# bdagnillo/altair-raytracing

Hardware: AMD Instinct MI355X
Metric: Mrays/sec whole-node, 180x90 fluxmap src(-60,0,-75); achieved HBM GB/s vs peak (higher is better)
Workload: dtype f64

## Files before the change

### altair-raytracing_amd/csrc/isx_api.hip

```cpp
#include "../../include/isx.h"
#include "isx_kernels.hpp"

#include <cmath>
#include <cstdio>
#include <cstdlib>
#include <cstring>
#include <algorithm>
#include <limits>
#include <map>
#include <new>
#include <tuple>
#include <variant>
#include <vector>

using namespace isx;

namespace {

struct State {
  bool init = false;
  int device = -1;
  int cu_count = 0;
  size_t lds_limit = 64 * 1024;
  hipStream_t stream = nullptr;
// ... 3178 lines not shown

int isx_scene_path_moments(const isx_scene_path_spec* pspec, const uint64_t* hist, const isx_scene_path_counts* counts,
                           double* mean_cm, double* sd_cm) {
  if (!pspec || !hist || !counts) return ISX_ERR_BAD_ARG;
  const int rc = check_scene_path_spec(pspec);
  if (rc) return rc;
  const size_t K = (size_t)pspec->n_bins;
  for (int f = 0; f < ISX_RESPONSE_FATES; ++f) {
    const uint64_t* row = hist + (size_t)f * K;
    double N = 0, A = 0, B = 0;
    for (size_t k = 0; k < K; ++k) {
      const double h = (double)row[k], x = ((double)k + 0.5) * pspec->bin_cm;
      N += h;
      A += x * h;
      B += x * x * h;
    }
    double m = std::numeric_limits<double>::quiet_NaN(), d = m;
    if (N > 0 && counts->overflow[f] == 0) {
      m = A / N;
      const double var = B / N - m * m;
      d = std::sqrt(var > 0 ? var : 0.0);
    }
    if (mean_cm) mean_cm[f] = m;
    if (sd_cm) sd_cm[f] = d;
  }
  return ISX_OK;
}

int isx_scene_path_decay(const isx_scene_path_spec* pspec, const uint64_t* hist, const isx_scene_path_counts* counts, int32_t f,
                         int32_t lo_bin, double* tau_cm, double* sigma_cm) {
  if (!pspec || !hist || !counts || !tau_cm || !sigma_cm) return ISX_ERR_BAD_ARG;
  const int rc = check_scene_path_spec(pspec);
  if (rc) return rc;
  if (f < 0 || f >= ISX_RESPONSE_FATES || lo_bin < 0 || lo_bin >= pspec->n_bins) return ISX_ERR_BAD_ARG;
  if (counts->overflow[f] != 0) return ISX_ERR_BAD_CONFIG;
  const uint64_t* row = hist + (size_t)f * (size_t)pspec->n_bins;
  double N = 0, Sm = 0;
  for (int32_t ib = lo_bin; ib < pspec->n_bins; ++ib) {
    const double h = (double)row[ib];
    Sm += (double)(ib - lo_bin) * h;
    N += h;
  }
  if (!(N > 0)) return ISX_ERR_BAD_CONFIG;
  const double m = Sm / N;
  if (!(m > 0)) return ISX_ERR_BAD_CONFIG;
  const double r = m / (1.0 + m);
  const double lr = std::log(r);
  *tau_cm = -pspec->bin_cm / lr;
  *sigma_cm = pspec->bin_cm / (lr * lr) / std::sqrt(N * m * (1.0 + m));
  return ISX_OK;
}

#ifdef ISX_DIAG
int isx_diag_read(uint64_t* out48) {
  if (!S.init || !out48) return ISX_ERR_BAD_ARG;
  if (trace_join()) return ISX_ERR_HIP;
  HIPCHK(hipStreamSynchronize(S.stream));
  HIPCHK(hipMemcpyFromSymbol(out48, HIP_SYMBOL(isx::g_diag), 48 * sizeof(unsigned long long)));
  unsigned long long z[48] = {0};
  HIPCHK(hipMemcpyToSymbol(HIP_SYMBOL(isx::g_diag), z, sizeof(z)));
  return ISX_OK;
}
#endif

}
```

### altair-raytracing_amd/csrc/isx_kernels.hpp

```cpp
#pragma once
#include <type_traits>
#include "isx_device.hpp"

namespace isx {

struct DetGrid {
  int n_theta, n_phi, nbins, bin_mode;
  int hit_line_mode, pad0;
  double half_w2;
  double rho_d;
  double R;
  double portz;
  const double* table;
  const double* rowtab;
  const double* coltab;
  const double* discs;
  double disc_r, disc_h;
  const float* clusters;
  const int* disc_perm;
  int n_clusters, pad1;
  uint64_t map_first, rays_per_group;
  int fold;
  int rec_stage;
  double* rec_lines;
  uint32_t* rec_counts;
  double* log_rec;
  unsigned long long* log_count;
  uint64_t log_cap;
  int xm_nu, xm_nv, xm_nx, xm_ny;
  double xm_plane_z, xm_half;
  unsigned long long* xm_dir;
  unsigned long long* xm_pos;
  unsigned long long* xm_counts;
};

#ifdef ISX_DIAG
__device__ unsigned long long g_diag[48];
#define ISX_DIAG_ADD(k, v) do { if (lane == 0) atomicAdd(&g_diag[k], (unsigned long long)(v)); } while (0)
#define ISX_DIAG_ADD_LANES(k, v) atomicAdd(&g_diag[k], (unsigned long long)(v))
#define ISX_TD_DECL unsigned long long td_[16] = {0}; unsigned long long tdc_ = clock64()
#define ISX_TD_MARK(k) do { const unsigned long long c_ = clock64(); td_[k] += c_ - tdc_; tdc_ = c_; } while (0)
#define ISX_TD_ADD(k, v) do { td_[k] += (unsigned long long)(v); } while (0)
#define ISX_TD_FLUSH() do { if (lane == 0) for (int k_ = 0; k_ < 16; ++k_) atomicAdd(&g_diag[16 + k_], td_[k_]); } while (0)
#define ISX_TD_FLUSH_AT(b_) do { if (lane == 0) for (int k_ = 0; k_ < 16; ++k_) atomicAdd(&g_diag[(b_) + k_], td_[k_]); } while (0)
#define ISX_BD_MARK(sq, k) do { if (lane == 0) { const unsigned long long c_ = clock64(); \
    const unsigned long long p_ = ((unsigned long long)(unsigned)(sq).head[7] << 32) | (unsigned)(sq).tail[7]; \
    atomicAdd(&g_diag[16 + (k)], c_ - p_); (sq).tail[7] = (int)(unsigned)c_; (sq).head[7] = (int)(unsigned)(c_ >> 32); } } while (0)
#define ISX_BD_INIT(sq) do { if (lane == 0) { const unsigned long long c_ = clock64(); (sq).tail[7] = (int)(unsigned)c_; (sq).head[7] = (int)(unsigned)(c_ >> 32); } } while (0)
#else
#define ISX_BD_INIT(sq) do { } while (0)
#define ISX_BD_MARK(sq, k) do { } while (0)
#define ISX_DIAG_ADD(k, v) do { } while (0)
#define ISX_DIAG_ADD_LANES(k, v) do { } while (0)
#define ISX_TD_DECL do { } while (0)
#define ISX_TD_MARK(k) do { } while (0)
#define ISX_TD_ADD(k, v) do { } while (0)
#define ISX_TD_FLUSH() do { } while (0)
#define ISX_TD_FLUSH_AT(b_) do { } while (0)
#endif

enum : int { SINK_FLUX = 0, SINK_DZ = 1, SINK_DISC = 2, SINK_PERPOS = 3, SINK_LOG = 4, SINK_DISCPOS = 5, SINK_REC = 6, SINK_EXITMAP = 7, SINK_WALL = 8,
              SINK_LIGHTFIELD = 9, SINK_ORDER = 10, SINK_PATCH = 11,
              SINK_RESPONSE = 12,
              SINK_VIEW = 13,
              SINK_FIELD = 14,
              SINK_SORDER = 15,
              SINK_SPATH = 16 };

struct Work {
  uint64_t seed, first, n;
  unsigned long long* hist;
  unsigned long long* stats;
  uint32_t* ctr;
  uint32_t sub, pad;
};
enum : int { Q_RAYS = 0 , Q_REGIONS = 2, Q_BIN = 3,
             Q_SCAN = 4 , Q_LIST = 6, Q_LISTB = 7, Q_WORDS = 8 };
constexpr uint32_t kRegion = 1024;

#ifndef ISX_BLOCK
#define ISX_BLOCK 1024
#endif
#ifndef ISX_WAVES_PER_EU
#define ISX_WAVES_PER_EU 0
#endif
constexpr int kBlock = ISX_BLOCK;
#ifndef ISX_ABL
#define ISX_ABL 0
#endif
#ifndef ISX_WALK4
#define ISX_WALK4 1
#endif
#ifndef ISX_ATOM_BRANCH
#define ISX_ATOM_BRANCH 0
#endif
#ifndef ISX_ASSIST_MIN
#define ISX_ASSIST_MIN 64
#endif
#ifndef ISX_ASSIST_LAZY
#define ISX_ASSIST_LAZY 128
#endif
// ... 651 lines not shown
        const int slot = lane >> logq;
        part = lane & ((1 << logq) - 1);
        have = slot < nlong;
        const int e = have ? ((volatile LdsInt*)split)[slot] : 0;
        owner = e & 63;
        i = e >> 8;
      }
      if (!have) i = 0;
      CapWin w;
      w.inv_dphi = inv_dphi;
      w.Fz = __shfl(pre.Fz, owner, 64); w.AF = __shfl(pre.AF, owner, 64); w.AF2 = w.AF * w.AF;
      w.jf = __shfl(pre.jf, owner, 64); w.ch2 = __shfl(pre.ch2, owner, 64);
      V3 P, V;
      {
        load_line(lines + 6 * owner, P, V);
      }
      int jlo = 0, cnt = 0;
      if (have) cap_window(w, (float)rowt[4 * i + 2], (float)rowt[4 * i + 3], d.n_phi, jlo, cnt);
      int start = 0, len = cnt;
      if (pass == 0) {
        const unsigned long long lm = __ballot(cnt > kSplitAt);
        if (lm != 0ull && __ballot(cnt >= kSplitAt + 16) != 0ull) {
          nlong = (int)__popcll(lm);
          logq = nlong <= 8 ? 3 : (nlong <= 16 ? 2 : (nlong <= 32 ? 1 : 0));
          if (logq > 0) {
            npass = 2;
            if (cnt > kSplitAt) {
              const uint32_t rank = __builtin_amdgcn_mbcnt_hi((uint32_t)(lm >> 32), __builtin_amdgcn_mbcnt_lo((uint32_t)lm, 0u));
              ((volatile LdsInt*)split)[rank] = owner | (i << 8);
              len = kSplitAt;
            }
            __builtin_amdgcn_wave_barrier();
          }
        }
      } else {
        const int rem = cnt - kSplitAt;
        const int chunk = (rem + (1 << logq) - 1) >> logq;
        start = kSplitAt + part * chunk;
        len = rem - part * chunk;
        len = len < 0 ? 0 : (len > chunk ? chunk : len);
        if (!have) len = 0;
      }
      ISX_DIAG_ADD(11, 1); if (pass == 1) ISX_DIAG_ADD(10, 1);
      const double t0 = -fma(P.x, V.x, fma(P.y, V.y, (P.z - d.portz) * V.z));
      walk_columns(d, hist, colx, P, V, t0, lane, i, rowt, jlo, start, len, 0, lines + 6 * owner);
    }
  }
}

constexpr int kClasses = 7, kQueueCap = 128;
constexpr int kSlotWaveWords = kClasses * kQueueCap + 16 + 64;
constexpr int kDeferCap = kDeferCapW;
constexpr int kDeferHead = 8;
constexpr int kColWaveWords = kClasses * kQueueCap + 16 + 64 + kDeferHead + kDeferCap;
constexpr int kPiece = 16, kLongest = 24;
struct SlotQueues {
  LdsWord* q;
  LdsInt* tail;
  LdsInt* head;
  const ColP* colp;
  LdsWord* defer;
};
__device__ __forceinline__ const uint2* defer_side(const SlotQueues& sq) {
  volatile LdsWord* df = sq.defer;
  return reinterpret_cast<const uint2*>((uintptr_t)((unsigned long long)df[1] | ((unsigned long long)df[2] << 32)));
}
__device__ __forceinline__ uint2 side_load(const uint2* side, int i) {
  const unsigned long long w = ((__attribute__((address_space(1))) const unsigned long long*)side)[i];
  return make_uint2((uint32_t)w, (uint32_t)(w >> 32));
}
__device__ __forceinline__ void redo_push(const SlotQueues& sq, uint32_t id, uint32_t bin) {
  volatile LdsWord* df = sq.defer;
  GlbU64* redo = (GlbU64*)(uintptr_t)((unsigned long long)df[4] | ((unsigned long long)df[5] << 32));
  const unsigned long long cap = (unsigned long long)df[6] | ((unsigned long long)df[7] << 32);
  const unsigned long long pos = __hip_atomic_fetch_add(redo, 1ull, __ATOMIC_RELAXED, __HIP_MEMORY_SCOPE_AGENT);
  if (pos < cap) redo[2ull + pos] = (unsigned long long)id | ((unsigned long long)bin << 32);
  else redo[1] = 1ull;
}
__device__ __forceinline__ int slot_class(int cnt) {
  return cnt <= 4 ? 0 : (cnt <= 12 ? (cnt - 3) >> 1 : (cnt <= 16 ? 5 : 6));
}

constexpr uint32_t kDeferFlushAt = 64;
template <class D>
__device__ __forceinline__ void flush_deferred(const D& d, uint32_t* __restrict__ hist, const double* __restrict__ rowt,
                                               const ColX* __restrict__ colx, const double* __restrict__ lines, const SlotQueues& sq,
                                               int lane) {
  volatile LdsWord* df = sq.defer;
  typedef __attribute__((address_space(3))) uint32_t LdsU32;
  const uint32_t held = df[0];
  const uint32_t n = held < (uint32_t)kDeferCap ? held : (uint32_t)kDeferCap;
#pragma unroll 1
  for (uint32_t base = 0; base < n; base += 64u) {
    const bool have = base + (uint32_t)lane < n;
    const uint32_t e = have ? df[(uint32_t)kDeferHead + base + (uint32_t)lane] : 0u;
    const int line = (int)(e & 255u), jr = (int)((e >> 8) & 255u), ir = (int)((e >> 16) & 255u);
    bool hit = false;
    const uint2* side = defer_side(sq);
    if (side) {
      uint2 se = make_uint2(0u, 0u);
      if (have) se = side_load(side, line);
      const float e = __uint_as_float(se.x);
      int res = 0;
      if (have) res = e > 0.f ? decide_approx(d, rowt, colx, lines + 6 * line, ir, jr, e) : (int)decide_exact(d, rowt, colx, lines + 6 * line, ir, jr);
      hit = res == 1;
      const unsigned long long rm = __ballot(res == 2);
      if (rm) {
// ... 147 lines not shown
  ilo = max((int)floorf((thF - omega) * k.inv_dth - 0.5f - 1e-3f), 0);
  ihi = min((int)ceilf((thF + omega) * k.inv_dth - 0.5f + 1e-3f), k.n_theta - 1);
  own.smax = Gz; own.smin = AF; own.vxy = phiF * k.inv_dphi - 0.5f; own.avz = ch2;
}

template <class D>
__device__ __forceinline__ void produce_rows_packed(const D& d, uint32_t* __restrict__ hist, const double* __restrict__ rowt,
                                                    const ColX* __restrict__ colx, const double* __restrict__ lines, const SlotQueues& sq,
                                                    const BoxLine& own, int own_ilo, int nrow, int excl, int incl, int total, bool boxes,
                                                    float inv_dphi, float portz, int first_line, int lane, LdsInt* mark) {
#pragma unroll 1
  for (int base = 0; base < total; base += 64) {
    const int g = base + lane;
    bool have = g < total;
    volatile LdsInt* mk = mark;
    mk[lane] = 0;
    __builtin_amdgcn_wave_barrier();
    if (nrow > 0 && excl < base + 64 && incl > base) mk[(excl > base ? excl : base) - base] = lane + 1;
    __builtin_amdgcn_wave_barrier();
    const int m = mk[lane];
    const unsigned long long low = __ballot(m != 0) & (~0ull >> (63 - lane));
    const int pos = 63 - __builtin_clzll(low | 1ull);
    int owner = mk[pos] - 1;
    if (!have || owner < 0) { owner = 0; have = false; }
    const int o_excl = __shfl(excl, owner, 64), o_ilo = __shfl(own_ilo, owner, 64);
    BoxLine b;
    b.smax = __shfl(own.smax, owner, 64); b.smin = __shfl(own.smin, owner, 64); b.vxy = __shfl(own.vxy, owner, 64);
    b.avz = __shfl(own.avz, owner, 64);
    b.ivz = b.dn = b.Hm = b.Hz = b.phin = b.rs = b.sig = 0.f;
    if (boxes) {
      b.ivz = __shfl(own.ivz, owner, 64); b.dn = __shfl(own.dn, owner, 64); b.Hm = __shfl(own.Hm, owner, 64);
      b.Hz = __shfl(own.Hz, owner, 64); b.phin = __shfl(own.phin, owner, 64); b.rs = __shfl(own.rs, owner, 64);
      b.sig = __shfl(own.sig, owner, 64);
    }
    const int i = have ? o_ilo + (g - o_excl) : 0;
    int j0 = 0, c0 = 0, j1 = 0, c1 = 0;
    if (have) {
      const float zi = (float)rowt[4 * i + 2], Ai = (float)rowt[4 * i + 3];
      if (boxes) box_window(b, zi - portz, Ai, d.n_phi, inv_dphi, j0, c0, j1, c1);
      else {
        CapWin w;
        w.inv_dphi = inv_dphi; w.Fz = b.smax; w.AF = b.smin; w.AF2 = b.smin * b.smin; w.jf = b.vxy; w.ch2 = b.avz;
        cap_window(w, zi, Ai, d.n_phi, j0, c0);
      }
    }
    const int nwin = (boxes && __ballot(c1 > 0) != 0ull) ? 2 : 1;
#pragma unroll 1
    for (int w = 0; w < nwin; ++w) push_slots(d, hist, rowt, colx, lines, sq, first_line + owner, i, w == 0 ? j0 : j1, w == 0 ? c0 : c1, lane);
  }
}

struct __align__(16) RowX { float S0, S1, C0, C1, T0, T1; uint32_t pad0, pad1; };
constexpr int kColPiece = 48, kColLongest = 64;
__device__ __forceinline__ int col_class(int cnt) { return cnt <= 48 ? (cnt - 1) >> 3 : 6; }

struct ColPre {
  float fx, fy, a, cosw;
  int jlo, ncol;
  int kind;
};
__device__ __forceinline__ ColPre prep_cols(const GridConst& k, int n_phi, const V3& P, const V3& V, const CapShared& sh, int side) {
  ColPre o;
  o.fx = o.fy = o.a = o.cosw = 0.f; o.jlo = 0; o.ncol = 0; o.kind = sh.kind;
  if (sh.kind != 0) return o;
  float Fx, Fy, mz;
  cap_centre(k, sh, P, V, side, Fx, Fy, mz);
  if (mz * sh.iL * k.Rf - sqrt_cull(cap_chord2(k, sh)) > 0.f) { o.kind = -3; return o; }
  o.fx = Fx * sh.iL; o.fy = Fy * sh.iL; o.a = -(mz * sh.iL);
  o.cosw = sh.cosw;
  o.kind = 0;
  const float sinF = sqrt_cull(fmaf(o.fx, o.fx, o.fy * o.fy));
  const float sinw = sqrt_cull(fmaxf(0.f, fmaf(-o.cosw, o.cosw, 1.0f)));
  if (!(sinF > sinw * 1.01f + 1e-4f)) { o.jlo = 0; o.ncol = n_phi; return o; }
  const float r = fminf(1.0f, sinw * rcp_cull(sinF) * 1.001f);
  const float dphi = (1.57079637f - acos_cull(r)) + 3e-3f;
  float phiF = atan2_cull(Fy, Fx);
  if (phiF < 0.f) phiF += 6.28318530718f;
  const float jc = phiF * k.inv_dphi - 0.5f, hw = dphi * k.inv_dphi + 0.02f;
  const int lo = (int)ceilf(jc - hw), hi = (int)floorf(jc + hw);
  int n = hi - lo + 1;
  if (n >= n_phi) { o.jlo = 0; o.ncol = n_phi; return o; }
  if (n < 0) n = 0;
  int j0 = lo;
  if (j0 < 0) j0 += n_phi;
  if (j0 >= n_phi) j0 -= n_phi;
  o.jlo = j0; o.ncol = n;
  return o;
}

__device__ __forceinline__ void cap_rows(float fx, float fy, float a, float cosw, float c32, float s32, float inv_dth, int n_theta,
                                         int& ilo, int& cnt) {
#if ISX_ABL == 3
  ilo = 20; cnt = 30; return;
#endif
  ilo = 0; cnt = 0;
  const float b = fmaf(c32, fx, s32 * fy);
  const float rho2 = fmaf(a, a, b * b);
  if (!(rho2 > 1e-12f)) { if (cosw < 1e-5f) cnt = n_theta; return; }
  const float x = cosw * __builtin_amdgcn_rsqf(rho2);
  if (x > 1.0f) return;
  if (x < 0.0f) { ilo = 0; cnt = n_theta; return; }
  const float dl = acos_cull(fmaxf(x, -1.0f)) + 2.5e-3f;
  const float tc = atan2_cull(b, a);
  const float tlo = tc - dl, thi = tc + dl;
  if (thi < 0.f || tlo > 1.57079637f) return;
  const int lo = max((int)ceilf(tlo * inv_dth - 0.5f - 1e-3f), 0);
  const int hi = min((int)floorf(thi * inv_dth - 0.5f + 1e-3f), n_theta - 1);
// ... 27 lines not shown
    ex = fmaf(-tv, Vx, tx); ey = fmaf(-tv, Vy, ty); ez = fmaf(-tv, Vz, tz);
    const float ie = __builtin_amdgcn_rsqf(fmaf(ex, ex, fmaf(ey, ey, ez * ez)));
    ex *= ie; ey *= ie; ez *= ie;
    cosw = -1.0f;
  }
  o.fx = ex; o.fy = ey; o.a = -ez; o.cosw = cosw; o.kind = 0;
  bp.ux = fmaf(Vy, ez, -(Vz * ey)); bp.uy = fmaf(Vz, ex, -(Vx * ez)); bp.uz = fmaf(Vx, ey, -(Vy * ex));
  bp.kap = fmaf(rs * iR, 1.0001f, 4e-6f) + kap_extra;
  const float sinF = sqrt_cull(fmaf(o.fx, o.fx, o.fy * o.fy));
  const float sinw = sqrt_cull(fmaxf(0.f, fmaf(-cosw, cosw, 1.0f)));
  if (!(cosw > 0.05f) || !(sinF > sinw * 1.01f + 1e-4f)) { o.jlo = 0; o.ncol = n_phi; return o; }
  const float r = fminf(1.0f, sinw * rcp_cull(sinF) * 1.001f);
  const float dphi = (1.57079637f - acos_cull(r)) + 3e-3f;
  float phiF = atan2_cull(o.fy, o.fx);
  if (phiF < 0.f) phiF += 6.28318530718f;
  const float jc = phiF * k.inv_dphi - 0.5f, hw = dphi * k.inv_dphi + 0.02f;
  const int lo = (int)ceilf(jc - hw), hi = (int)floorf(jc + hw);
  int n = hi - lo + 1;
  if (n >= n_phi) { o.jlo = 0; o.ncol = n_phi; return o; }
  if (n < 0) n = 0;
  int j0 = lo;
  if (j0 < 0) j0 += n_phi;
  if (j0 >= n_phi) j0 -= n_phi;
  o.jlo = j0; o.ncol = n;
  return o;
}
__device__ __forceinline__ void band_rows(const BandPre& bp, float c32, float s32, float inv_dth, int row_lo, int row_hi, int& ilo, int& cnt,
                                          int& ilo_b, int& cnt_b) {
  ilo = cnt = ilo_b = cnt_b = 0;
  if (row_hi < row_lo) return;
  const float ga = fmaf(c32, bp.ux, s32 * bp.uy);
  const float N2 = fmaf(ga, ga, bp.uz * bp.uz);
  if (!(N2 > bp.kap * bp.kap * 1.03f + 1e-12f)) { ilo = row_lo; cnt = row_hi - row_lo + 1; return; }
  const float x = bp.kap * __builtin_amdgcn_rsqf(N2);
  const float al = (1.57079637f - acos_cull(x)) + 2.6e-3f;
  const float de = atan2_cull(bp.uz, ga);
#pragma unroll
  for (int m = -1; m <= 1; ++m) {
    const float ce = fmaf((float)m, 3.14159274f, de);
    const float tlo = ce - al, thi = ce + al;
    if (thi < 0.f || tlo > 1.57079637f) continue;
    const int lo = max((int)ceilf(tlo * inv_dth - 0.5f - 1e-3f), row_lo);
    const int hi = min((int)floorf(thi * inv_dth - 0.5f + 1e-3f), row_hi);
    if (hi < lo) continue;
    if (cnt == 0) { ilo = lo; cnt = hi - lo + 1; }
    else { ilo_b = lo; cnt_b = hi - lo + 1; }
  }
}

template <class D>
__device__ __forceinline__ void consume_cols(const D& d, uint32_t* __restrict__ hist, const double* __restrict__ rowt,
                                             const ColX* __restrict__ colx, const RowX* __restrict__ rowx,
                                             const double* __restrict__ lines, uint32_t rec, bool active, int lane,
                                             const SlotQueues& sq) {
  ISX_BD_MARK(sq, 3);
#if ISX_ABL == 2
  return;
#endif
  const int line = (int)(rec & 255u), j = (int)((rec >> 8) & 255u), ilo = (int)((rec >> 16) & 255u);
  const int len = active ? (int)(rec >> 24) : 0;
  const double* src6 = lines + 6 * line;
  float cAl = 0.f, cBe = 0.f, cVz = 0.f, cQz = 0.f, cE0 = 0.f, cE1 = 0.f, cE2 = 0.f, cF0 = 0.f, cF1 = 0.f, cF2 = 0.f;
  float band32 = 0.f;
  if (len > 0) {
    V3 P, V;
    {
      load_line(src6, P, V);
    }
    const double wz = P.z - d.portz;
    const double t0 = -fma(P.x, V.x, fma(P.y, V.y, wz * V.z));
    const double qx = fma(t0, V.x, P.x), qy = fma(t0, V.y, P.y), qz = fma(t0, V.z, wz);
    const double cph = colx[j].c, sph = colx[j].s;
    const double al = fma(V.y, cph, -(V.x * sph)), be = fma(qy, cph, -(qx * sph));
    const double ga = fma(V.x, cph, V.y * sph), de = fma(qx, cph, qy * sph);
    const double R = d.R, R2x = 2.0 * R;
    const double e0 = -2.0 * fma(qx, V.x, fma(qy, V.y, qz * V.z));
    const double f0 = fma(qx, qx, fma(qy, qy, fma(qz, qz, R * R))) - d.half_w2;
    const double e1 = R2x * ga, e2 = -(R2x * V.z), f1 = -(R2x * de), f2 = R2x * qz;
    cAl = (float)al; cBe = (float)be; cVz = (float)(-V.z); cQz = (float)(-qz);
    cE0 = (float)e0; cF0 = (float)f0; cE1 = (float)e1; cF1 = (float)f1; cE2 = (float)e2; cF2 = (float)f2;
    const double Md = fabs(al) + fabs(V.z), Mn = fabs(be) + (fabs(qz) + R);
    const double Mv = fabs(e0) + (fabs(e1) + fabs(e2)), Mf = fabs(f0) + (fabs(f1) + fabs(f2));
    const double Sg = fma(Md, fma(Md, Mf, Mn * Mv), Mn * Mn);
    band32 = Sg >= 1e-6 ? (float)(1.4e-6 * Sg) * 1.000001f + 1e-30f : __builtin_inff();
    const uint32_t ub = ((volatile LdsWord*)sq.defer)[3];
    if (ub) {
      const float tg = (float)(fma(Mn, Mn + Mv, Mf) + d.half_w2);
      const float er = __uint_as_float(ub) * rcp_cull((float)R) * 1.0001f;
      band32 = er <= 1e-3f ? fmaf(1.001f, band32, (13.8f * er) * tg) : __builtin_inff();
    }
  }
  typedef __attribute__((address_space(3))) uint32_t LdsU32;
  typedef __attribute__((address_space(3))) unsigned char LdsByte;
  const uint32_t row_bytes = (uint32_t)d.n_phi * 4u;
  LdsByte* bin = reinterpret_cast<LdsByte*>((__attribute__((address_space(3))) void*)hist) + (uint32_t)j * 4u + (uint32_t)ilo * row_bytes;
#if !ISX_WALK4
  const RowX* rp = rowx + ilo;
#endif
  const isx_f2 vAl = {cAl, cAl}, vBe = {cBe, cBe}, vVz = {cVz, cVz}, vQz = {cQz, cQz}, vE0 = {cE0, cE0}, vE1 = {cE1, cE1},
               vE2 = {cE2, cE2}, vF0 = {cF0, cF0}, vF1 = {cF1, cF1}, vF2 = {cF2, cF2};
  if (len > 0) ISX_DIAG_ADD_LANES(7, len);
  ISX_DIAG_ADD(11, 1);
  ISX_BD_MARK(sq, 4);
#if ISX_ABL == 1
  if (band32 == 12345.f) hist[0] = (uint32_t)(cAl + cBe + cVz + cQz + cE0 + cE1 + cE2 + cF0 + cF1 + cF2);
  return;
#endif
// ... 11 lines not shown
    const isx_f2 ddw = __builtin_elementwise_fma(vF1, SS, __builtin_elementwise_fma(vF2, CC, vF0));
    const isx_f2 g = __builtin_elementwise_fma(dot, __builtin_elementwise_fma(dot, ddw, num * mdv), num * num);
    bool hit0 = g.x < 0.f, hit1 = g.y < 0.f;
    if (one && !(fminf(fabsf(g.x), fabsf(g.y)) > band32)) {
#pragma unroll 1
      for (int t = 0; t < 2; ++t) {
        const float gt = t == 0 ? g.x : g.y;
        if (fabsf(gt) > band32 || (t == 1 && !two)) continue;
#ifndef ISX_DIAG_TIMING_ONLY
        ISX_DIAG_ADD_LANES(12, 1);
#endif
        int ir = ilo + kk + t;
        asm volatile("" : "+v"(ir));
        bool hit = false;
        typedef __attribute__((address_space(3))) uint32_t LdsCnt;
#if defined(ISX_DIAG) && !defined(ISX_DIAG_TIMING_ONLY)
        const uint32_t pos = (uint32_t)kDeferCap;
#else
        const uint32_t pos = __hip_atomic_fetch_add(reinterpret_cast<LdsCnt*>(sq.defer), 1u, __ATOMIC_RELAXED, __HIP_MEMORY_SCOPE_WORKGROUP);
#endif
        if (pos < (uint32_t)kDeferCap) {
          ((volatile LdsWord*)sq.defer)[(uint32_t)kDeferHead + pos] = (uint32_t)line | ((uint32_t)j << 8) | ((uint32_t)ir << 16);
        } else {
          int jr = j;
          asm volatile("" : "+v"(jr));
          uint2 se = make_uint2(0u, 0u);
          const uint2* side = defer_side(sq);
          if (side) se = side_load(side, line + (jr - j));
          if (__uint_as_float(se.x) > 0.f) redo_push(sq, se.y, (uint32_t)(ir * d.n_phi + jr));
          else hit = decide_exact(d, rowt, colx, src6 + (jr - j), ir, jr);
        }
        if (t == 0) hit0 = hit; else hit1 = hit;
      }
    }
    h0 = hit0 && one;
    h1 = hit1 && two;
#if defined(ISX_DIAG) && !defined(ISX_DIAG_TIMING_ONLY)
    {
      V3 P, V;
      load_line(src6, P, V);
      for (int t = 0; t < (two ? 2 : (one ? 1 : 0)); ++t) {
        const bool ref = check_intersection(d.table + 6 * (size_t)((ilo + kk + t) * d.n_phi + j), d.half_w2, P, V);
        if (ref != (t == 0 ? h0 : h1)) ISX_DIAG_ADD_LANES(14, 1);
      }
    }
#endif
  };
  int ie = ilo;
  for (int k = 0;; k += 4) {
    const bool act = k < len;
    if (__ballot(act) == 0ull) break;
#ifndef ISX_DIAG_TIMING_ONLY
    ISX_DIAG_ADD(4, 4);
#endif
    if (act) {
      bool a0, a1, b0, b1;
#if ISX_ABL == 5
      classify((k & 3), k, a0, a1);
      classify(2 + (k & 3), k + 2, b0, b1);
#else
      classify(ie, k, a0, a1);
      classify(ie + 2, k + 2, b0, b1);
#endif
      ie += 4;
#ifdef ISX_DIAG_MULT
      {
        const bool hs[4] = {a0, a1, b0, b1};
        for (int t = 0; t < 4; ++t) {
          const uint32_t addr = (uint32_t)(uintptr_t)(bin + (uint32_t)t * row_bytes);
          const unsigned long long hm = __ballot(hs[t]);
          bool dup = false;
          unsigned long long mm = hm;
          while (mm) {
            const int sl = __builtin_ctzll(mm);
            mm &= mm - 1ull;
            const uint32_t a2 = (uint32_t)__builtin_amdgcn_readlane((int)addr, sl);
            if (hs[t] && sl < lane && a2 == addr) dup = true;
          }
          const int n_add = (int)__popcll(hm), n_dup = (int)__popcll(__ballot(dup));
          ISX_DIAG_ADD(8, n_add); ISX_DIAG_ADD(9, n_dup);
        }
      }
#endif
#if ISX_ATOM_BRANCH
      if (a0) __hip_atomic_fetch_add(reinterpret_cast<LdsU32*>(bin), 1u, __ATOMIC_RELAXED, __HIP_MEMORY_SCOPE_WORKGROUP);
      if (a1) __hip_atomic_fetch_add(reinterpret_cast<LdsU32*>(bin + row_bytes), 1u, __ATOMIC_RELAXED, __HIP_MEMORY_SCOPE_WORKGROUP);
      if (b0) __hip_atomic_fetch_add(reinterpret_cast<LdsU32*>(bin + 2u * row_bytes), 1u, __ATOMIC_RELAXED, __HIP_MEMORY_SCOPE_WORKGROUP);
      if (b1) __hip_atomic_fetch_add(reinterpret_cast<LdsU32*>(bin + 3u * row_bytes), 1u, __ATOMIC_RELAXED, __HIP_MEMORY_SCOPE_WORKGROUP);
#else
#if ISX_ABL == 4
      if (a0 && a1 && b0 && b1 && band32 == 12345.f)
#endif
      __hip_atomic_fetch_add(reinterpret_cast<LdsU32*>(bin), a0 ? 1u : 0u, __ATOMIC_RELAXED, __HIP_MEMORY_SCOPE_WORKGROUP);
#if ISX_ABL == 4
      if (a0 && a1 && b0 && b1 && band32 == 12345.f) {
#endif
      __hip_atomic_fetch_add(reinterpret_cast<LdsU32*>(bin + row_bytes), a1 ? 1u : 0u, __ATOMIC_RELAXED, __HIP_MEMORY_SCOPE_WORKGROUP);
      __hip_atomic_fetch_add(reinterpret_cast<LdsU32*>(bin + 2u * row_bytes), b0 ? 1u : 0u, __ATOMIC_RELAXED, __HIP_MEMORY_SCOPE_WORKGROUP);
      __hip_atomic_fetch_add(reinterpret_cast<LdsU32*>(bin + 3u * row_bytes), b1 ? 1u : 0u, __ATOMIC_RELAXED, __HIP_MEMORY_SCOPE_WORKGROUP);
#if ISX_ABL == 4
      }
#endif
#endif
      bin += 4u * row_bytes;
    }
  }
// ... 27 lines not shown
          int ir = ilo + k + t;
          asm volatile("" : "+v"(ir));
          bool hit = false;
          {
            const double sd = rowt[4 * ir + 0], cd = rowt[4 * ir + 1], zz = rowt[4 * ir + 2], ad = rowt[4 * ir + 3];
            int jr = j;
            asm volatile("" : "+v"(jr));
            const double cph = colx[jr].c, sph = colx[jr].s;
            V3 P, V;
            {
              load_line(src6 + (jr - j), P, V);
            }
            const double pz = P.z - zz;
            const double dotd = fma(sd * V.y, cph, fma(-(sd * V.x), sph, -(cd * V.z)));
            const double numd = fma(sd * P.y, cph, fma(-(sd * P.x), sph, -(cd * pz)));
            const double m2dv = fma(2.0 * (ad * V.x), cph, fma(2.0 * (ad * V.y), sph, -2.0 * fma(P.x, V.x, fma(P.y, V.y, pz * V.z))));
            const double f0 = fma(P.x, P.x, fma(P.y, P.y, fma(ad, ad, pz * pz)));
            const double f1c = -2.0 * (ad * P.x), f2c = -2.0 * (ad * P.y);
            const double ddwd = fma(f1c, cph, fma(f2c, sph, f0 - d.half_w2));
            const double diff = fma(dotd, fma(dotd, ddwd, numd * m2dv), numd * numd);
            const double bandc = 2.1e-9 * fma(2.0, f0 + (fabs(f1c) + fabs(f2c)), d.half_w2);
            hit = diff < 0.0;
            if (fabs(dotd) < 1e-4 || fabs(diff) <= bandc) {
              ISX_DIAG_ADD_LANES(13, 1);
              const double* tab = d.table;
              asm volatile("" : "+v"(tab));
              hit = check_intersection(tab + 6 * (size_t)(ir * d.n_phi + jr), d.half_w2, P, V);
            }
          }
          if (t == 0) hit0 = hit; else hit1 = hit;
        }
      }
      hit1 = hit1 && two;
#if defined(ISX_DIAG) && !defined(ISX_DIAG_TIMING_ONLY)
      {
        V3 P, V;
        load_line(src6, P, V);
        for (int t = 0; t < (two ? 2 : 1); ++t) {
          const bool ref = check_intersection(d.table + 6 * (size_t)((ilo + k + t) * d.n_phi + j), d.half_w2, P, V);
          if (ref != (t == 0 ? hit0 : hit1)) ISX_DIAG_ADD_LANES(14, 1);
        }
      }
#endif
      rp += 2;
      __hip_atomic_fetch_add(reinterpret_cast<LdsU32*>(bin), hit0 ? 1u : 0u, __ATOMIC_RELAXED, __HIP_MEMORY_SCOPE_WORKGROUP);
      __hip_atomic_fetch_add(reinterpret_cast<LdsU32*>(bin + row_bytes), hit1 ? 1u : 0u, __ATOMIC_RELAXED, __HIP_MEMORY_SCOPE_WORKGROUP);
      bin += 2u * row_bytes;
    }
  }
#endif
  ISX_BD_MARK(sq, 5);
}

template <class D>
__device__ __forceinline__ void drain_cols(const D& d, uint32_t* __restrict__ hist, const double* __restrict__ rowt,
                                           const ColX* __restrict__ colx, const RowX* __restrict__ rowx,
                                           const double* __restrict__ lines, const SlotQueues& sq, int least, int lane) {
  volatile LdsInt* tl = sq.tail;
  volatile LdsInt* hd = sq.head;
  const int held = lane < kClasses ? tl[lane] - hd[lane] : 0;
  unsigned long long m = __ballot(held >= least);
  while (m) {
    const int c = __builtin_ctzll(m);
    m &= m - 1ull;
    const int h = hd[c], n = tl[c] - h;
    const int take = n < 64 ? n : 64;
    const uint32_t rec = lane < take ? ((volatile LdsWord*)sq.q)[c * kQueueCap + ((h + lane) & (kQueueCap - 1))] : 0u;
    __builtin_amdgcn_wave_barrier();
    if (lane == 0) hd[c] = h + take;
    __builtin_amdgcn_wave_barrier();
    consume_cols(d, hist, rowt, colx, rowx, lines, rec, lane < take, lane, sq);
  }
}

template <class D>
__device__ __forceinline__ void push_cols(const D& d, uint32_t* __restrict__ hist, const double* __restrict__ rowt,
                                          const ColX* __restrict__ colx, const RowX* __restrict__ rowx,
                                          const double* __restrict__ lines, const SlotQueues& sq, int line, int j, int ilo, int cnt,
                                          int lane) {
  int i0 = ilo, rem = cnt;
  ISX_BD_MARK(sq, 1);
  for (;;) {
    const int piece = rem > kColLongest ? kColPiece : rem;
    if (piece > 0) {
      const int c = col_class(piece);
      const int pos = __hip_atomic_fetch_add(sq.tail + c, 1, __ATOMIC_RELAXED, __HIP_MEMORY_SCOPE_WORKGROUP);
      ((volatile LdsWord*)sq.q)[c * kQueueCap + (pos & (kQueueCap - 1))] =
          (uint32_t)line | ((uint32_t)j << 8) | ((uint32_t)i0 << 16) | ((uint32_t)piece << 24);
    }
    rem -= piece;
    i0 += piece;
    __builtin_amdgcn_wave_barrier();
    ISX_BD_MARK(sq, 2);
    drain_cols(d, hist, rowt, colx, rowx, lines, sq, 64, lane);
    if (__ballot(rem > 0) == 0ull) break;
  }
}

template <class D>
__device__ __forceinline__ void produce_cols_packed(const D& d, uint32_t* __restrict__ hist, const double* __restrict__ rowt,
                                                    const ColX* __restrict__ colx, const RowX* __restrict__ rowx,
                                                    const double* __restrict__ lines, const SlotQueues& sq, const ColPre& pre,
                                                    int excl, int incl, int total, float inv_dth, int n_theta, int first_line,
                                                    int lane, LdsInt* mark, const BandPre& bp, bool band) {
#pragma unroll 1
  for (int base = 0; base < total; base += 64) {
    const int g = base + lane;
    bool have = g < total;
    ISX_BD_MARK(sq, 9);
    volatile LdsInt* mk = mark;
    mk[lane] = 0;
    __builtin_amdgcn_wave_barrier();
    if (pre.ncol > 0 && excl < base + 64 && incl > base) mk[(excl > base ? excl : base) - base] = lane + 1;
    __builtin_amdgcn_wave_barrier();
    const int m = mk[lane];
    const unsigned long long low = __ballot(m != 0) & (~0ull >> (63 - lane));
    const int pos = 63 - __builtin_clzll(low | 1ull);
    int owner = mk[pos] - 1;
    if (!have || owner < 0) { owner = 0; have = false; }
    ISX_BD_MARK(sq, 6);
    const int o_excl = __shfl(excl, owner, 64), o_jlo = __shfl(pre.jlo, owner, 64);
    const float fx = __shfl(pre.fx, owner, 64), fy = __shfl(pre.fy, owner, 64), a = __shfl(pre.a, owner, 64), cw = __shfl(pre.cosw, owner, 64);
    ISX_BD_MARK(sq, 7);
    int j = o_jlo + (g - o_excl);
    if (j >= d.n_phi) j -= d.n_phi;
    if (!have) j = 0;
    int ilo = 0, cnt = 0, ilo_b = 0, cnt_b = 0;
    const float c32 = colx[j].c32, s32 = colx[j].s32;
    if (have) cap_rows(fx, fy, a, cw, c32, s32, inv_dth, n_theta, ilo, cnt);
    if (band) {
      BandPre ob;
      ob.ux = __shfl(bp.ux, owner, 64); ob.uy = __shfl(bp.uy, owner, 64); ob.uz = __shfl(bp.uz, owner, 64); ob.kap = __shfl(bp.kap, owner, 64);
      const int r_lo = ilo, r_hi = ilo + cnt - 1;
      band_rows(ob, c32, s32, inv_dth, r_lo, have ? r_hi : r_lo - 1, ilo, cnt, ilo_b, cnt_b);
    }
    const int npiece = (band && __ballot(cnt_b > 0) != 0ull) ? 2 : 1;
#pragma unroll 1
    for (int w = 0; w < npiece; ++w)
      push_cols(d, hist, rowt, colx, rowx, lines, sq, first_line + owner, j, w == 0 ? ilo : ilo_b, w == 0 ? cnt : cnt_b, lane);
  }
}

__device__ __forceinline__ void hit_line_compat(V3& P, V3& V) {
  const double dx = P.x - 0.0, dy = P.y - 0.0, dz = P.z - 0.0;
  const double mag = sqrt(dx * dx + dy * dy + dz * dz);
  const double ex = dx / mag, ey = dy / mag, ez = dz / mag;
  const double m2 = sqrt(ex * ex + ey * ey + ez * ez);
// ... 2617 lines not shown
  unsigned long long* ghist = wk.hist;
  asm volatile("" : "+s"(ghist));
  for (int b = tid; b < nbins; b += nthr) {
    const uint32_t c = hist[b];
    if (c) { global_add_u64(&ghist[b], (unsigned long long)c); flushed += c; }
  }
  if (flushed) atomicAdd(&wk.stats[5], flushed);
}

extern "C" __global__ void __launch_bounds__(kBlock) __attribute__((amdgpu_waves_per_eu(ISX_BIN_WAVES_PER_EU, ISX_BIN_WAVES_PER_EU)))
isx_bin_cols_kernel(const DetGrid d_arg, const Work wk) {
  extern __shared__ __align__(16) unsigned char smem[];
  uint32_t* hist = reinterpret_cast<uint32_t*>(smem);
  const int nbins = d_arg.nbins;
  const size_t off_row = ((size_t)nbins * 4 + 15) & ~(size_t)15;
  double* rowt = reinterpret_cast<double*>(smem + off_row);
  ColX* colx = reinterpret_cast<ColX*>(rowt + 4 * d_arg.n_theta);
  RowX* rowx = reinterpret_cast<RowX*>(colx + 2 * d_arg.n_phi);
  DetGrid* d_lds = reinterpret_cast<DetGrid*>(rowx + d_arg.n_theta + 4);
  uint32_t* wave_all = reinterpret_cast<uint32_t*>(d_lds + 1);
  const int tid = threadIdx.x, lane = tid & 63;
  const int nthr = (int)blockDim.x;
  for (int b = tid; b < nbins; b += nthr) hist[b] = 0u;
  for (int b = tid; b < 4 * d_arg.n_theta; b += nthr) rowt[b] = d_arg.rowtab[b];
  for (int b = tid; b <= d_arg.n_theta; b += nthr) {
    RowX e;
    e.S0 = e.S1 = e.C0 = e.C1 = e.T0 = e.T1 = 0.f; e.pad0 = e.pad1 = 0u;
    if (b < d_arg.n_theta) {
      const double sd = d_arg.rowtab[4 * b], cd = d_arg.rowtab[4 * b + 1];
      e.S0 = (float)sd; e.C0 = (float)cd; e.T0 = (float)(-(d_arg.R * (cd * cd)));
    }
    if (b + 1 < d_arg.n_theta) {
      const double sd = d_arg.rowtab[4 * b + 4], cd = d_arg.rowtab[4 * b + 5];
      e.S1 = (float)sd; e.C1 = (float)cd; e.T1 = (float)(-(d_arg.R * (cd * cd)));
    }
#if ISX_WALK4
    reinterpret_cast<float4*>(rowx)[b] = make_float4(e.S0, e.S1, e.C0, e.C1);
    reinterpret_cast<float2*>(reinterpret_cast<float4*>(rowx) + (d_arg.n_theta + 4))[b] = make_float2(e.T0, e.T1);
#else
    rowx[b] = e;
#endif
  }
  for (int b = tid; b < 2 * d_arg.n_phi; b += nthr) {
    const int j = b < d_arg.n_phi ? b : b - d_arg.n_phi;
    ColX e;
    e.c = d_arg.coltab[2 * j]; e.s = d_arg.coltab[2 * j + 1]; e.off4 = (uint32_t)j * 4u; e.c32 = (float)e.c; e.s32 = (float)e.s; e.pad = 0u;
    colx[b] = e;
  }
  if (tid == (nthr > 128 ? 128 : 0)) *d_lds = d_arg;
  uint32_t* mine = wave_all + (size_t)(tid >> 6) * kColWaveWords;
  SlotQueues sq;
  sq.colp = nullptr;
  sq.q = (LdsWord*)mine;
  sq.tail = (LdsInt*)(mine + kClasses * kQueueCap);
  sq.head = sq.tail + 8;
  LdsInt* mrk = sq.head + 8;
  sq.defer = (LdsWord*)(mrk + 64);
  if (lane < 16) sq.tail[lane] = 0;
  if (lane == 0) {
    const unsigned long long rp = (unsigned long long)(uintptr_t)d_arg.log_count, rcap = d_arg.log_cap;
    sq.defer[0] = 0u; sq.defer[1] = 0u; sq.defer[2] = 0u; sq.defer[3] = 0u;
    sq.defer[4] = (uint32_t)rp; sq.defer[5] = (uint32_t)(rp >> 32); sq.defer[6] = (uint32_t)rcap; sq.defer[7] = (uint32_t)(rcap >> 32);
  }
  __syncthreads();
  typedef __attribute__((address_space(3))) DetGrid LdsDetGrid;
  const volatile LdsDetGrid& d = *(const volatile LdsDetGrid*)d_lds;

  const uint32_t n_regions = wk.ctr[Q_REGIONS];
  const uint32_t ushift = 2u + wk.pad;
  ISX_BD_INIT(sq);
#pragma unroll 1
  for (;;) {
    uint32_t unit = 0;
    if (lane == 0) unit = atomicAdd(&wk.ctr[Q_BIN], 1u);
    unit = (uint32_t)__builtin_amdgcn_readfirstlane((int)unit);
    const uint32_t region = unit >> ushift;
    if (region >= n_regions) break;
    const uint32_t r_word = (uint32_t)__builtin_amdgcn_readfirstlane((int)d_arg.rec_counts[region]);
    const uint32_t r_lines = (r_word >> 31) ? (r_word & 0x7ffu) : r_word;
    const uint32_t q_first = (unit & ((1u << ushift) - 1u)) * (kRegion >> ushift);
    const uint32_t n_lines = r_lines < q_first + (kRegion >> ushift) ? r_lines : q_first + (kRegion >> ushift);
    const double* lines = d_arg.rec_lines + 6ull * ((uint64_t)region * kRegion + q_first);
    {
      const unsigned long long sp = (r_word >> 31) ? (unsigned long long)(uintptr_t)(reinterpret_cast<const uint2*>(d_arg.log_rec) + ((uint64_t)region * kRegion + q_first)) : 0ull;
      if (lane == 0) { sq.defer[1] = (uint32_t)sp; sq.defer[2] = (uint32_t)(sp >> 32); sq.defer[3] = (r_word >> 31) ? (r_word & 0x7ffff800u) : 0u; }
      __builtin_amdgcn_wave_barrier();
    }
    struct { int n_phi, n_theta; double half_w2, portz, R; const double* table; } dcol;
    dcol.n_phi = d.n_phi; dcol.n_theta = d.n_theta; dcol.half_w2 = d.half_w2; dcol.portz = d_arg.portz; dcol.R = d_arg.R; dcol.table = d.table;
#pragma unroll 1
    for (uint32_t b0 = q_first; b0 < n_lines; b0 += 64u) {
      const bool have = b0 + (uint32_t)lane < n_lines;
      const int first_line = (int)(b0 - q_first);
      unsigned long long m_second = 0ull, m_band = 0ull;
#pragma unroll 1
      for (int pass = 0; pass < 3; ++pass) {
        const unsigned long long pm = pass == 0 ? __ballot(have) : (pass == 1 ? m_second : m_band);
        if (pm == 0ull) continue;
        const bool part = ((pm >> lane) & 1ull) != 0ull;
        ColPre pre;
        pre.fx = pre.fy = pre.a = pre.cosw = 0.f; pre.jlo = 0; pre.ncol = 0; pre.kind = -2;
        BandPre bp;
        bp.ux = bp.uy = bp.uz = 0.f; bp.kap = 2.f;
        bool low2 = false, graze = false;
        if (part) {
          GridConst k;
          k.Rf = (float)d.R; k.rho = (float)d.rho_d; k.portz = (float)d.portz; k.n_theta = d.n_theta;
          k.inv_dphi = (float)d.n_phi * 0.15915494309f;
          k.inv_dth = 0.f;
          uint32_t li = (uint32_t)(first_line + lane);
          asm volatile("" : "+v"(li));
          V3 lp, lv;
          load_line(lines + 6 * li, lp, lv);
          if (pass < 2) {
            CapShared sh = prep_shared(k, lp, lv);
            if (pass == 0 && sh.kind == 0) {
              low2 = cap_is_low(k, sh, lp, lv, 1);
              if (low2 && caps_may_touch(k, sh)) { sh.kind = -1; low2 = false; }
            }
            graze = sh.kind == -1;
            pre = prep_cols(k, dcol.n_phi, lp, lv, sh, pass);
          } else {
            pre = prep_band(k, dcol.n_phi, lp, lv, bp);
          }
        }
        if (pass == 0) {
          ISX_BD_MARK(sq, 0);
          m_second = __ballot(low2);
          m_band = __ballot(graze);
          { const int n_fast = (int)__popcll(__ballot(part && pre.kind == 0 && pre.ncol > 0)); (void)n_fast; ISX_DIAG_ADD(0, n_fast); }
        }
        if (pass == 2) { const int n_box = (int)__popcll(__ballot(part && pre.kind == 0)); (void)n_box; ISX_DIAG_ADD(2, n_box); }
        { const int n_far = (int)__popcll(__ballot(part && pre.kind == -2)); (void)n_far; ISX_DIAG_ADD(3, n_far); }
        const int ncol = (part && pre.kind == 0) ? pre.ncol : 0;
        int incl = ncol;
#pragma unroll
        for (int dlt = 1; dlt < 64; dlt <<= 1) {
          const int o = __shfl_up(incl, dlt, 64);
          if (lane >= dlt) incl += o;
        }
        const int total = __builtin_amdgcn_readlane(incl, 63);
        if (total == 0) continue;
        ColPre pc = pre;
        pc.ncol = ncol;
        const int n_theta = d.n_theta;
        produce_cols_packed(dcol, hist, rowt, colx, rowx, lines, sq, pc, incl - ncol, incl, total, (float)n_theta * 0.63661977237f, n_theta,
                            first_line, lane, mrk, bp, pass == 2);
      }
      if (((volatile LdsWord*)sq.defer)[0] >= kDeferFlushAt) flush_deferred(dcol, hist, rowt, colx, lines, sq, lane);
    }
    drain_cols(dcol, hist, rowt, colx, rowx, lines, sq, 1, lane);
    flush_deferred(dcol, hist, rowt, colx, lines, sq, lane);
  }
  __syncthreads();
  unsigned long long flushed = 0;
  unsigned long long* ghist = wk.hist;
  asm volatile("" : "+s"(ghist));
  for (int b = tid; b < nbins; b += nthr) {
    const uint32_t c = hist[b];
    if (c) { global_add_u64(&ghist[b], (unsigned long long)c); flushed += c; }
  }
  if (flushed) atomicAdd(&wk.stats[5], flushed);
}

#ifndef ISX_SCAN_BLOCKS
#define ISX_SCAN_BLOCKS 4
#endif
constexpr int kScanBlocks = ISX_SCAN_BLOCKS;
constexpr int kScanBlock = 256;
#ifndef ISX_SCAN_SUB
#define ISX_SCAN_SUB 2048
#endif
#ifndef ISX_SCAN_BATCH
#define ISX_SCAN_BATCH 512
#endif
constexpr uint32_t kScanSub = ISX_SCAN_SUB;
constexpr uint32_t kScanBatch = ISX_SCAN_BATCH;
struct FateScan {
  FateConsts f;
  uint64_t seed, first;
  uint32_t n, pairs;
  uint32_t* list;
  uint32_t* ctr;
  unsigned long long* stats;
};
extern "C" __global__ void __launch_bounds__(kScanBlock)
isx_fate_scan_kernel(const FateScan a) {
  __shared__ unsigned long long s_cen[2];
  __shared__ uint32_t s_batch[kScanBlock / 64][kScanBatch + 64];
  __shared__ uint16_t s_stop[kScanBlock / 64][kScanBatch + 64];
  const int tid = threadIdx.x, lane = tid & 63;
  if (tid < 2) s_cen[tid] = 0ull;
  __syncthreads();
  typedef __attribute__((address_space(3))) uint32_t LdsU32;
  typedef __attribute__((address_space(3))) uint16_t LdsU16;
  volatile LdsU32* batch = (volatile LdsU32*)s_batch[__builtin_amdgcn_readfirstlane(tid >> 6)];
  volatile LdsU16* stop = (volatile LdsU16*)s_stop[__builtin_amdgcn_readfirstlane(tid >> 6)];
  uint32_t n_batch = 0;
  auto flush_batch = [&]() {
    uint32_t base = 0;
    if (lane == 0) base = atomicAdd(a.ctr + Q_LIST, n_batch);
    base = (uint32_t)__builtin_amdgcn_readfirstlane((int)base);
    __builtin_amdgcn_wave_barrier();
    if (a.pairs) {
// ... 478 lines not shown
```

Before: 5162.

## Refine column queue classes and pack mixed-class leftovers in end drain

Doubles the number of column-length classes to 13, each with 64-entry LDS queues, so that records in a drained batch have more similar lengths and less lane divergence. Pushes now retry when a queue is full and drains fire only on a full 64-entry queue. The final drain packs leftovers from all classes into full 64-lane batches using a prefix scan, instead of draining each class separately with partial waves. The diagnostic buffer and clock-stamp slots are moved to fit the new layout. The added bookkeeping and bounded push retries cost extra instructions, and leftover batches now mix record lengths.

```diff
diff --git a/altair-raytracing_amd/csrc/isx_api.hip b/altair-raytracing_amd/csrc/isx_api.hip
--- a/altair-raytracing_amd/csrc/isx_api.hip
+++ b/altair-raytracing_amd/csrc/isx_api.hip
@@ -3254,12 +3254,12 @@
 }
 
 #ifdef ISX_DIAG
-int isx_diag_read(uint64_t* out48) {
-  if (!S.init || !out48) return ISX_ERR_BAD_ARG;
+int isx_diag_read(uint64_t* out64) {
+  if (!S.init || !out64) return ISX_ERR_BAD_ARG;
   if (trace_join()) return ISX_ERR_HIP;
   HIPCHK(hipStreamSynchronize(S.stream));
-  HIPCHK(hipMemcpyFromSymbol(out48, HIP_SYMBOL(isx::g_diag), 48 * sizeof(unsigned long long)));
-  unsigned long long z[48] = {0};
+  HIPCHK(hipMemcpyFromSymbol(out64, HIP_SYMBOL(isx::g_diag), 64 * sizeof(unsigned long long)));
+  unsigned long long z[64] = {0};
   HIPCHK(hipMemcpyToSymbol(HIP_SYMBOL(isx::g_diag), z, sizeof(z)));
   return ISX_OK;
 }
diff --git a/altair-raytracing_amd/csrc/isx_kernels.hpp b/altair-raytracing_amd/csrc/isx_kernels.hpp
--- a/altair-raytracing_amd/csrc/isx_kernels.hpp
+++ b/altair-raytracing_amd/csrc/isx_kernels.hpp
@@ -35,7 +35,7 @@
 };
 
 #ifdef ISX_DIAG
-__device__ unsigned long long g_diag[48];
+__device__ unsigned long long g_diag[64];
 #define ISX_DIAG_ADD(k, v) do { if (lane == 0) atomicAdd(&g_diag[k], (unsigned long long)(v)); } while (0)
 #define ISX_DIAG_ADD_LANES(k, v) atomicAdd(&g_diag[k], (unsigned long long)(v))
 #define ISX_TD_DECL unsigned long long td_[16] = {0}; unsigned long long tdc_ = clock64()
@@ -43,10 +43,12 @@
 #define ISX_TD_ADD(k, v) do { td_[k] += (unsigned long long)(v); } while (0)
 #define ISX_TD_FLUSH() do { if (lane == 0) for (int k_ = 0; k_ < 16; ++k_) atomicAdd(&g_diag[16 + k_], td_[k_]); } while (0)
 #define ISX_TD_FLUSH_AT(b_) do { if (lane == 0) for (int k_ = 0; k_ < 16; ++k_) atomicAdd(&g_diag[(b_) + k_], td_[k_]); } while (0)
+#define ISX_BD_LO(sq) (sq).head[-1]
+#define ISX_BD_HI(sq) (sq).head[(int)((sq).head - (sq).tail) - 1]
 #define ISX_BD_MARK(sq, k) do { if (lane == 0) { const unsigned long long c_ = clock64(); \
-    const unsigned long long p_ = ((unsigned long long)(unsigned)(sq).head[7] << 32) | (unsigned)(sq).tail[7]; \
-    atomicAdd(&g_diag[16 + (k)], c_ - p_); (sq).tail[7] = (int)(unsigned)c_; (sq).head[7] = (int)(unsigned)(c_ >> 32); } } while (0)
-#define ISX_BD_INIT(sq) do { if (lane == 0) { const unsigned long long c_ = clock64(); (sq).tail[7] = (int)(unsigned)c_; (sq).head[7] = (int)(unsigned)(c_ >> 32); } } while (0)
+    const unsigned long long p_ = ((unsigned long long)(unsigned)ISX_BD_HI(sq) << 32) | (unsigned)ISX_BD_LO(sq); \
+    atomicAdd(&g_diag[16 + (k)], c_ - p_); ISX_BD_LO(sq) = (int)(unsigned)c_; ISX_BD_HI(sq) = (int)(unsigned)(c_ >> 32); } } while (0)
+#define ISX_BD_INIT(sq) do { if (lane == 0) { const unsigned long long c_ = clock64(); ISX_BD_LO(sq) = (int)(unsigned)c_; ISX_BD_HI(sq) = (int)(unsigned)(c_ >> 32); } } while (0)
 #else
 #define ISX_BD_INIT(sq) do { } while (0)
 #define ISX_BD_MARK(sq, k) do { } while (0)
@@ -804,7 +806,9 @@
 constexpr int kSlotWaveWords = kClasses * kQueueCap + 16 + 64;
 constexpr int kDeferCap = kDeferCapW;
 constexpr int kDeferHead = 8;
-constexpr int kColWaveWords = kClasses * kQueueCap + 16 + 64 + kDeferHead + kDeferCap;
+constexpr int kColClasses = 13, kColQueueCap = 64;
+constexpr int kColPushTurns = 2 * (1 + (256 + 47) / 48);
+constexpr int kColWaveWords = kColClasses * kColQueueCap + 32 + 64 + kDeferHead + kDeferCap;
 constexpr int kPiece = 16, kLongest = 24;
 struct SlotQueues {
   LdsWord* q;
@@ -1058,7 +1062,7 @@
 
 struct __align__(16) RowX { float S0, S1, C0, C1, T0, T1; uint32_t pad0, pad1; };
 constexpr int kColPiece = 48, kColLongest = 64;
-__device__ __forceinline__ int col_class(int cnt) { return cnt <= 48 ? (cnt - 1) >> 3 : 6; }
+__device__ __forceinline__ int col_class(int cnt) { return cnt <= 48 ? (cnt - 1) >> 2 : kColClasses - 1; }
 
 struct ColPre {
   float fx, fy, a, cosw;
@@ -1192,7 +1196,8 @@
 __device__ __forceinline__ void consume_cols(const D& d, uint32_t* __restrict__ hist, const double* __restrict__ rowt,
                                              const ColX* __restrict__ colx, const RowX* __restrict__ rowx,
                                              const double* __restrict__ lines, uint32_t rec, bool active, int lane,
-                                             const SlotQueues& sq) {
+                                             const SlotQueues& sq, bool at_end) {
+  (void)at_end;
   ISX_BD_MARK(sq, 3);
 #if ISX_ABL == 2
   return;
@@ -1310,6 +1315,7 @@
     if (__ballot(act) == 0ull) break;
 #ifndef ISX_DIAG_TIMING_ONLY
     ISX_DIAG_ADD(4, 4);
+    if (at_end) ISX_DIAG_ADD(15, 4);
 #endif
     if (act) {
       bool a0, a1, b0, b1;
@@ -1443,24 +1449,55 @@
   ISX_BD_MARK(sq, 5);
 }
 
+
 template <class D>
 __device__ __forceinline__ void drain_cols(const D& d, uint32_t* __restrict__ hist, const double* __restrict__ rowt,
                                            const ColX* __restrict__ colx, const RowX* __restrict__ rowx,
-                                           const double* __restrict__ lines, const SlotQueues& sq, int least, int lane) {
+                                           const double* __restrict__ lines, const SlotQueues& sq, int lane) {
   volatile LdsInt* tl = sq.tail;
   volatile LdsInt* hd = sq.head;
-  const int held = lane < kClasses ? tl[lane] - hd[lane] : 0;
-  unsigned long long m = __ballot(held >= least);
+  const int held = lane < kColClasses ? tl[lane] - hd[lane] : 0;
+  unsigned long long m = __ballot(held >= kColQueueCap);
   while (m) {
     const int c = __builtin_ctzll(m);
     m &= m - 1ull;
-    const int h = hd[c], n = tl[c] - h;
-    const int take = n < 64 ? n : 64;
-    const uint32_t rec = lane < take ? ((volatile LdsWord*)sq.q)[c * kQueueCap + ((h + lane) & (kQueueCap - 1))] : 0u;
+    const int h = hd[c];
+    const uint32_t rec = ((volatile LdsWord*)sq.q)[c * kColQueueCap + ((h + lane) & (kColQueueCap - 1))];
     __builtin_amdgcn_wave_barrier();
-    if (lane == 0) hd[c] = h + take;
+    if (lane == 0) hd[c] = h + kColQueueCap;
     __builtin_amdgcn_wave_barrier();
-    consume_cols(d, hist, rowt, colx, rowx, lines, rec, lane < take, lane, sq);
+    consume_cols(d, hist, rowt, colx, rowx, lines, rec, true, lane, sq, false);
+  }
+}
+
+template <class D>
+__device__ __forceinline__ void drain_cols_end(const D& d, uint32_t* __restrict__ hist, const double* __restrict__ rowt,
+                                               const ColX* __restrict__ colx, const RowX* __restrict__ rowx,
+                                               const double* __restrict__ lines, const SlotQueues& sq, int lane) {
+  volatile LdsInt* tl = sq.tail;
+  volatile LdsInt* hd = sq.head;
+  const int h_own = lane < kColClasses ? hd[lane] : 0;
+  const int held = lane < kColClasses ? tl[lane] - h_own : 0;
+  int incl = held;
+#pragma unroll
+  for (int dlt = 1; dlt < 16; dlt <<= 1) {
+    const int o = __shfl_up(incl, dlt, 64);
+    if (lane >= dlt) incl += o;
+  }
+  const int total = __builtin_amdgcn_readlane(incl, kColClasses - 1);
+  __builtin_amdgcn_wave_barrier();
+  if (lane < kColClasses) hd[lane] = h_own + held;
+  __builtin_amdgcn_wave_barrier();
+#pragma unroll 1
+  for (int base = 0; base < total; base += 64) {
+    const int g = base + lane;
+    const bool act = g < total;
+    int c = 0;
+#pragma unroll
+    for (int k = 0; k < kColClasses - 1; ++k) c += __builtin_amdgcn_readlane(incl, k) <= g ? 1 : 0;
+    const int first = __shfl(incl - held, c, 64), h = __shfl(h_own, c, 64);
+    const uint32_t rec = act ? ((volatile LdsWord*)sq.q)[c * kColQueueCap + ((h + (g - first)) & (kColQueueCap - 1))] : 0u;
+    consume_cols(d, hist, rowt, colx, rowx, lines, rec, act, lane, sq, true);
   }
 }
 
@@ -1470,20 +1507,28 @@
                                           const double* __restrict__ lines, const SlotQueues& sq, int line, int j, int ilo, int cnt,
                                           int lane) {
   int i0 = ilo, rem = cnt;
+  int pos = -1;
   ISX_BD_MARK(sq, 1);
-  for (;;) {
+#pragma unroll 1
+  for (int turn = 0; turn < kColPushTurns; ++turn) {
     const int piece = rem > kColLongest ? kColPiece : rem;
     if (piece > 0) {
       const int c = col_class(piece);
-      const int pos = __hip_atomic_fetch_add(sq.tail + c, 1, __ATOMIC_RELAXED, __HIP_MEMORY_SCOPE_WORKGROUP);
-      ((volatile LdsWord*)sq.q)[c * kQueueCap + (pos & (kQueueCap - 1))] =
-          (uint32_t)line | ((uint32_t)j << 8) | ((uint32_t)i0 << 16) | ((uint32_t)piece << 24);
-    }
-    rem -= piece;
-    i0 += piece;
+      if (pos < 0) {
+        ISX_DIAG_ADD_LANES(48 + c, 1);
+        pos = __hip_atomic_fetch_add(sq.tail + c, 1, __ATOMIC_RELAXED, __HIP_MEMORY_SCOPE_WORKGROUP);
+      }
+      if (pos - ((volatile LdsInt*)sq.head)[c] < kColQueueCap) {
+        ((volatile LdsWord*)sq.q)[c * kColQueueCap + (pos & (kColQueueCap - 1))] =
+            (uint32_t)line | ((uint32_t)j << 8) | ((uint32_t)i0 << 16) | ((uint32_t)piece << 24);
+        rem -= piece;
+        i0 += piece;
+        pos = -1;
+      }
+    }
     __builtin_amdgcn_wave_barrier();
     ISX_BD_MARK(sq, 2);
-    drain_cols(d, hist, rowt, colx, rowx, lines, sq, 64, lane);
+    drain_cols(d, hist, rowt, colx, rowx, lines, sq, lane);
     if (__ballot(rem > 0) == 0ull) break;
   }
 }
@@ -4207,11 +4252,11 @@
   SlotQueues sq;
   sq.colp = nullptr;
   sq.q = (LdsWord*)mine;
-  sq.tail = (LdsInt*)(mine + kClasses * kQueueCap);
-  sq.head = sq.tail + 8;
-  LdsInt* mrk = sq.head + 8;
+  sq.tail = (LdsInt*)(mine + kColClasses * kColQueueCap);
+  sq.head = sq.tail + 16;
+  LdsInt* mrk = sq.head + 16;
   sq.defer = (LdsWord*)(mrk + 64);
-  if (lane < 16) sq.tail[lane] = 0;
+  if (lane < 32) sq.tail[lane] = 0;
   if (lane == 0) {
     const unsigned long long rp = (unsigned long long)(uintptr_t)d_arg.log_count, rcap = d_arg.log_cap;
     sq.defer[0] = 0u; sq.defer[1] = 0u; sq.defer[2] = 0u; sq.defer[3] = 0u;
@@ -4304,7 +4349,7 @@
       }
       if (((volatile LdsWord*)sq.defer)[0] >= kDeferFlushAt) flush_deferred(dcol, hist, rowt, colx, lines, sq, lane);
     }
-    drain_cols(dcol, hist, rowt, colx, rowx, lines, sq, 1, lane);
+    drain_cols_end(dcol, hist, rowt, colx, rowx, lines, sq, lane);
     flush_deferred(dcol, hist, rowt, colx, lines, sq, lane);
   }
   __syncthreads();
```

After: 5188, median of 6. Within noise of the previous version (+0.5%).
